# AIM-SE/AC-TSR

Hardware: AMD Instinct MI355X
Metric: user-sequences/sec fwd+bwd, AC-SASRec L=50 d=64, 1/2/4/8 MI355X (higher is better)
Workload: dtype f32; 1 GPU; ACSASRec full training step (spatial + adversarial calibrators, BASELINE configs[2]), synthetic 100000-item catalogue, B=512/GPU L=50 d=64 h=2 2 layers inner=256, CE loss, two-pass backward + Adam; global_batch=512, seq_len=50, hidden=64, heads=2, parallelism=dp1, launch=hipGraph replay per step, backward=two walks (reference protocol, trainer.py:672-686)

## Files before the change

### ac_tsr_amd/_lib.py

```python
from __future__ import annotations

import ctypes as C
import os
import subprocess

_HERE = os.path.dirname(os.path.abspath(__file__))
CSRC = os.path.join(_HERE, "csrc")
LIB_PATH = os.environ.get("ACATTN_LIB") or os.path.join(CSRC, "libacattn.so")
HEADER_PATH = os.path.join(os.path.dirname(_HERE), "include", "acattn.h")

ABI_VERSION = 29
MAX_MASKS = 8
NSTAT = 8
MASK_STRUCTURED, MASK_DENSE_LL, MASK_DENSE_L = 0, 1, 2
COMBINE = {"fixed": 0, "gate": 1, "annealing": 2}
RICH = {"none": 0, "fixed": 1, "trainable": 2}
RNG_EXPLICIT, RNG_COUNTER = 0, 1
FWD_AUTO, FWD_STREAM, FWD_STAGED, FWD_GENERAL = 0, 1, 2, 3
BWD_AUTO, BWD_STREAM, BWD_ROW = 0, 1, 2

_f = C.c_void_p


class Problem(C.Structure):
    _fields_ = [
        ("B", C.c_int32), ("L", C.c_int32), ("H", C.c_int32), ("n_heads", C.c_int32),
        ("q", _f), ("k", _f), ("v", _f), ("qa", _f), ("ka", _f), ("gate_logits", _f),
        ("mask_mode", C.c_int32), ("causal", C.c_int32), ("key_valid", _f), ("mask", _f),
        ("w_order", _f), ("b_order", _f), ("w_dist", _f), ("b_dist", _f), ("scalar", _f),
        ("adversarial", C.c_int32), ("combine_option", C.c_int32), ("anneal_rate", C.c_float),
        ("two_level", C.c_int32), ("rich_combine", C.c_int32), ("rich_ratio", _f),
        ("rng_mode", C.c_int32), ("p_drop", C.c_float), ("noise", _f), ("keep_after", _f), ("keep_before", _f),
        ("keep_mask", _f), ("seed", C.c_uint64), ("seed_device", _f), ("affine", _f), ("gate_is_prob", C.c_int32),
    ]


class FwdOut(C.Structure):
    _fields_ = [
        ("ctx_attacked", _f), ("ctx_calibrated", _f), ("attack_mask", _f), ("row_stats", _f),
        ("after_spatial", _f), ("before_spatial", _f), ("perturbed_attention", _f), ("calibrated_attention", _f),
        ("penalty_part", _f),
    ]


# ... 63 lines not shown


class TailBwdIO(C.Structure):
    _fields_ = [("d_out", _f), ("d_ctx", _f), ("d_x", _f), ("d_h1", _f), ("d_h2", _f), ("d_h3", _f), ("dgb_part", _f),
                ("workspace", _f)]


class EmbedProblem(C.Structure):
    _fields_ = [("rows", C.c_int32), ("L", C.c_int32), ("H", C.c_int32), ("n_table_rows", C.c_int64), ("idx", _f),
                ("table", _f), ("pos", _f), ("gamma", _f), ("beta", _f), ("eps", C.c_float), ("p_drop", C.c_float),
                ("keep", _f), ("seed", C.c_uint64), ("seed_device", _f), ("nonzero_out", _f), ("hot_id_plus1", C.c_int64)]


EMBED_BWD_CHUNKS = 8
PENALTY_WS_FLOATS = 1024
WGRAD_MAX_GROUP = 8
WGRAD_MAX_REDUCE = 32
SUMROWS_MAX_DEFER = 8

SYMBOLS = {
    "acattn_abi_version": (C.c_int, []),
    "acattn_calibrated_attention_bwd_gate_summed": (C.c_int, [C.POINTER(Problem), C.POINTER(BwdIO)]),
    "acattn_calibrated_attention_bwd_pair_supported": (C.c_int, [C.POINTER(Problem), C.POINTER(BwdIO)]),
    "acattn_last_error": (C.c_char_p, []),
    "acattn_fwd_algorithmic_bytes": (C.c_int64, [C.POINTER(Problem)]),
    "acattn_calibrated_attention_fwd": (C.c_int, [C.POINTER(Problem), C.POINTER(FwdOut), C.c_void_p]),
    "acattn_calibrated_attention_bwd": (C.c_int, [C.POINTER(Problem), C.POINTER(BwdIO), C.c_void_p]),
    "acattn_spatial_affines": (C.c_int, [C.POINTER(Problem), _f, C.c_void_p]),
    "acattn_full_sort_ce_workspace_bytes": (C.c_int64, [C.POINTER(CeProblem)]),
    "acattn_full_sort_ce_fwd": (C.c_int, [C.POINTER(CeProblem), _f, _f, _f, C.c_void_p]),
    "acattn_full_sort_ce_fwd_dir": (C.c_int, [C.POINTER(CeProblem), _f, _f, _f, _f, C.c_void_p]),
    "acattn_full_sort_ce_bwd": (C.c_int, [C.POINTER(CeProblem), _f, _f, _f, _f, _f, C.c_void_p]),
    "acattn_full_sort_ce_products": (C.c_int, [C.c_int]),
    "acattn_dropout_add_layernorm_fwd": (C.c_int, [C.POINTER(LnProblem), _f, _f, C.c_void_p]),
    "acattn_dropout_add_layernorm_bwd": (C.c_int, [C.POINTER(LnProblem), _f, _f, _f, _f, _f, C.c_void_p]),
    "acattn_embed_layernorm_fwd": (C.c_int, [C.POINTER(EmbedProblem), _f, _f, C.c_void_p]),
    "acattn_embed_layernorm_bwd": (C.c_int, [C.POINTER(EmbedProblem), _f, _f, C.c_int64, _f, _f, _f, C.c_void_p]),
    "acattn_projections_supported": (C.c_int, [C.c_int32, C.c_int32]),
    "acattn_projections_bwd_workspace_bytes": (C.c_int64, [C.POINTER(ProjProblem)]),
    "acattn_projections_fwd": (C.c_int, [C.POINTER(ProjProblem), C.POINTER(ProjOut), C.c_void_p]),
    "acattn_projections_bwd": (C.c_int, [C.POINTER(ProjProblem), C.POINTER(ProjBwdIO), C.c_void_p]),
    "acattn_layer_tail_supported": (C.c_int, [C.c_int32, C.c_int32]),
    "acattn_layer_tail_fwd": (C.c_int, [C.POINTER(TailProblem), C.POINTER(TailSaved), C.c_void_p]),
    "acattn_layer_tail_bwd": (C.c_int, [C.POINTER(TailProblem), C.POINTER(TailSaved), C.POINTER(TailBwdIO), C.c_void_p]),
    "acattn_layer_tail_bwd_partial_rows": (C.c_int32, [C.c_int32]),
    "acattn_layer_tail_bwd_partial_rows_for": (C.c_int32, [C.c_int32, C.c_int32]),
    "acattn_layer_tail_bwd_workspace_bytes": (C.c_int64, [C.c_int32, C.c_int32]),
    "acattn_select_layer_tail_blocks": (C.c_int, [C.c_int]),
    "acattn_adam_step": (C.c_int, [C.POINTER(AdamGroup), C.c_double, C.c_double, C.c_double, C.c_double, C.c_double, _f,
                                   C.c_void_p]),
    "acattn_dense_ce_fwd": (C.c_int, [_f, C.c_int64, C.c_int64, _f, _f, _f, C.c_void_p]),
    "acattn_dense_ce_bwd": (C.c_int, [_f, _f, _f, _f, C.c_int64, C.c_int64, _f, C.c_void_p]),
    "acattn_step_inputs": (C.c_int, [C.POINTER(C.c_void_p), C.POINTER(C.c_void_p), C.POINTER(C.c_int64), C.c_int32, C.c_void_p,
                                     C.c_void_p, C.c_void_p, C.c_int32, C.c_void_p]),
    "acattn_sum_rows": (C.c_int, [_f, _f, C.c_int32, C.c_int32, C.c_int32, C.c_void_p]),
    "acattn_sum_rows_pair": (C.c_int, [_f, _f, C.c_int32, C.c_int32, C.c_int32, _f, _f, C.c_int32, C.c_int32, C.c_int32, C.c_void_p]),
    "acattn_mask_penalty_fwd": (C.c_int, [_f, C.c_int64, _f, _f, C.c_void_p]),
    "acattn_mask_penalty_partial": (C.c_int, [_f, C.c_int64, _f, C.c_void_p]),
    "acattn_mask_penalty_partial_multi": (C.c_int, [C.c_void_p, C.c_int32, C.c_int64, _f, C.c_void_p]),
    "acattn_mask_penalty_bwd_scaled_multi": (C.c_int, [C.c_void_p, _f, _f, C.c_float, C.c_int64, C.c_void_p, C.c_int32,
                                                       C.c_void_p]),
    "acattn_attacked_loss_finish": (C.c_int, [_f, C.c_int32, _f, C.c_int32, C.c_int64, C.c_float, _f, _f, C.c_int32,
                                              C.c_void_p]),
    "acattn_mask_penalty_rows": (C.c_int, [_f, C.c_int32, C.c_int32, C.c_int32, _f, C.c_void_p]),
    "acattn_attacked_loss_finish_rows": (C.c_int, [_f, C.c_int32, C.c_void_p, C.c_int32, C.c_int32, C.c_float, _f, _f, C.c_int32,
                                                  C.c_void_p]),
# ... 65 lines not shown
```

### ac_tsr_amd/csrc/acattn_api.hip

```cpp
#include <stdint.h>
#include <stdio.h>
#include <string.h>

#include <algorithm>

#include "acattn_common.h"

namespace {
thread_local char g_err[256] = "";

int fail(const char* msg) {
  snprintf(g_err, sizeof(g_err), "%s", msg);
  return -1;
}

int check_problem(const acattn_problem* p) {
  if (!p) return fail("problem is NULL");
  if (p->B < 1 || p->L < 1 || p->H < 1 || p->n_heads < 1) return fail("B, L, H, n_heads must be positive");
  if (p->H % p->n_heads != 0)
    return fail("The hidden size is not a multiple of the number of attention heads");
  const int dh = p->H / p->n_heads;
  if (dh != 16 && dh != 32 && dh != 64 && dh != 128) return fail("unsupported head size: dh must be 16, 32, 64 or 128");
  if (p->L > 208) return fail("unsupported sequence length: L must be <= 208");
  if (!p->q || !p->k || !p->v) return fail("q, k, v must be non-NULL");
// ... 126 lines not shown
int64_t acattn_full_sort_ce_workspace_bytes(const acattn_ce_problem* p) {
  if (!p || (p->H != 64 && p->H != 128 && p->H != 256)) return -1;
  return acattn_ce_ws_bytes(*p);
}

int acattn_full_sort_ce_fwd(const acattn_ce_problem* p, void* workspace, float* lse, float* row_loss, void* stream) {
  if (int rc = check_ce(p)) return rc;
  if (!workspace || !lse || !row_loss) return fail("workspace, lse, row_loss must be non-NULL");
  const int rc = acattn_launch_ce_fwd(*p, workspace, lse, row_loss, (hipStream_t)stream);
  if (rc > 0) snprintf(g_err, sizeof(g_err), "HIP launch failed: %s", hipGetErrorString((hipError_t)rc));
  return rc;
}

int acattn_full_sort_ce_fwd_dir(const acattn_ce_problem* p, void* workspace, float* lse, float* row_loss, float* dir,
                                void* stream) {
  if (int rc = check_ce(p)) return rc;
  if (!workspace || !lse || !row_loss || !dir) return fail("workspace, lse, row_loss, dir must be non-NULL");
  const int rc = acattn_launch_ce_fwd_dir(*p, workspace, lse, row_loss, dir, (hipStream_t)stream);
  if (rc > 0) snprintf(g_err, sizeof(g_err), "HIP launch failed: %s", hipGetErrorString((hipError_t)rc));
  return rc;
}

int acattn_full_sort_ce_bwd(const acattn_ce_problem* p, const float* lse, const float* coef, void* workspace,
                            float* d_out, float* d_table, void* stream) {
  if (int rc = check_ce(p)) return rc;
  if (!workspace || !lse || !coef || !d_out) return fail("workspace, lse, coef, d_out must be non-NULL");
  const int rc = acattn_launch_ce_bwd(*p, lse, coef, workspace, d_out, d_table, (hipStream_t)stream);
  if (rc > 0) snprintf(g_err, sizeof(g_err), "HIP launch failed: %s", hipGetErrorString((hipError_t)rc));
  return rc;
}

int acattn_full_sort_ce_products(int mode) { return acattn_ce_products_choice(mode); }

static int check_ln(const acattn_ln_problem* p) {
  if (!p) return fail("ln problem is NULL");
  if (p->rows < 1) return fail("rows must be positive");
  if (p->H != 64 && p->H != 128 && p->H != 256) return fail("unsupported hidden size for the fused LayerNorm: H must be 64, 128 or 256");
  if (p->residual_rows < 1 || p->rows % p->residual_rows != 0) return fail("residual_rows must divide rows");
  if (!p->z || !p->residual || !p->gamma || !p->beta) return fail("z, residual, gamma, beta must be non-NULL");
  if (p->p_drop < 0.f || p->p_drop >= 1.f) return fail("p_drop must lie in [0, 1)");
  return 0;
}

int acattn_dropout_add_layernorm_fwd(const acattn_ln_problem* p, float* y, float* stats, void* stream) {
  if (int rc = check_ln(p)) return rc;
  if (!y || !stats) return fail("y and stats must be non-NULL");
  const int rc = acattn_launch_ln_fwd(*p, y, stats, (hipStream_t)stream);
  if (rc > 0) snprintf(g_err, sizeof(g_err), "HIP launch failed: %s", hipGetErrorString((hipError_t)rc));
  return rc;
}

int acattn_dropout_add_layernorm_bwd(const acattn_ln_problem* p, const float* dy, const float* stats, float* dz,
                                     float* dres, float* dgb_part, void* stream) {
  if (int rc = check_ln(p)) return rc;
  if (!dy || !stats) return fail("dy and stats must be non-NULL");
  const int rc = acattn_launch_ln_bwd(*p, dy, stats, dz, dres, dgb_part, (hipStream_t)stream);
  if (rc > 0) snprintf(g_err, sizeof(g_err), "HIP launch failed: %s", hipGetErrorString((hipError_t)rc));
  return rc;
}

static int check_proj(const acattn_proj_problem* p) {
  if (!p) return fail("problem must be non-NULL");
  if (p->rows < 1) return fail("rows must be positive");
  if (!acattn_proj_supported(p->H, p->G)) return fail("projections: hidden_size must be 64, 128 or 256 and the gate at most 256 wide");
  if (!p->x || !p->wq || !p->bq || !p->wk || !p->bk || !p->wv || !p->bv || !p->waq || !p->baq || !p->wak || !p->bak)
    return fail("projections: input and parameters must be non-NULL");
// ... 363 lines not shown
```

### ac_tsr_amd/csrc/acattn_ce_bf16.hip

```cpp
#include <stdlib.h>

#include "acattn_common.h"

namespace {

constexpr float kLog2e = 1.44269504088896340736f;
constexpr float kLn2 = 0.69314718055994530942f;
constexpr int CH = 64;
constexpr int NW = 4;
constexpr int ES = CH + 4;
constexpr int HSLOTS = 24;
constexpr int HB_BYTES = HSLOTS * 64 * 16;
#ifndef CE6_EC_AGPR
#define CE6_EC_AGPR 1
#endif
#ifndef CE6_PIPE
#define CE6_PIPE 0
#endif

typedef __bf16 b8 __attribute__((ext_vector_type(8)));
typedef __bf16 b4 __attribute__((ext_vector_type(4)));
typedef short s4v __attribute__((ext_vector_type(4)));
typedef short s8v __attribute__((ext_vector_type(8)));

#define CE6_TERMS(X) X(0, 2) X(1, 1) X(2, 0) X(0, 1) X(1, 0) X(0, 0)

__device__ __forceinline__ f4 mfma_bf(const b8 a, const b8 b, const f4 c) {
  return __builtin_amdgcn_mfma_f32_16x16x32_bf16(a, b, c, 0, 0, 0);
}

__device__ __forceinline__ void dma16(const void* gsrc, void* lds_dst) {
  const uint32_t lds_off = (uint32_t)(uintptr_t)(__attribute__((address_space(3))) char*)lds_dst;
  asm volatile("s_mov_b32 m0, %1\n\ts_nop 0\n\tglobal_load_lds_dwordx4 %0, off" ::"v"(gsrc), "s"(lds_off) : "memory", "m0");
}

__device__ __forceinline__ void split8(const float (&x)[8], b8& p0, b8& p1, b8& p2) {
#pragma unroll
  for (int j = 0; j < 8; ++j) {
    const __bf16 a = (__bf16)x[j];
    const float r1 = x[j] - (float)a;
    const __bf16 b = (__bf16)r1;
    const float r2 = r1 - (float)b;
    p0[j] = a;
    p1[j] = b;
    p2[j] = (__bf16)r2;
  }
}

__global__ void __launch_bounds__(256) ce_split_rows_kernel(const float* __restrict__ out, const int B, b8* __restrict__ Hb,
                                                            float* __restrict__ zero, const int64_t n_zero) {
  const int sb = blockIdx.x;
  for (int64_t i = (int64_t)blockIdx.x * 256 + threadIdx.x; i < n_zero; i += (int64_t)gridDim.x * 256) zero[i] = 0.f;
  for (int e = threadIdx.x; e < 8 * 64; e += 256) {
    const int grp = e >> 6, lane = e & 63, c = lane & 15, g = lane >> 4;
    float x[8];
    if (grp < 4) {
      const int row = 32 * sb + 16 * (grp >> 1) + c;
      f4 v0 = {0.f, 0.f, 0.f, 0.f}, v1 = v0;
      if (row < B) {
        v0 = *(const f4*)(out + (size_t)row * CH + 32 * (grp & 1) + 8 * g);
        v1 = *(const f4*)(out + (size_t)row * CH + 32 * (grp & 1) + 8 * g + 4);
      }
#pragma unroll
      for (int j = 0; j < 4; ++j) {
        x[j] = v0[j];
        x[4 + j] = v1[j];
      }
    } else {
#pragma unroll
      for (int j = 0; j < 8; ++j) {
        const int row = 32 * sb + 8 * g + j;
        x[j] = row < B ? out[(size_t)row * CH + 16 * (grp - 4) + c] : 0.f;
      }
    }
    b8 p[3];
    split8(x, p[0], p[1], p[2]);
#pragma unroll
    for (int q = 0; q < 3; ++q) {
      const int slot = grp < 4 ? grp * 3 + q : 12 + 4 * q + (grp - 4);
// ... 828 lines not shown
```

### ac_tsr_amd/csrc/acattn_common.h

```cpp
#pragma once
#include <hip/hip_runtime.h>
#include <stdint.h>

#include <type_traits>

#include "acattn.h"

typedef float f4 __attribute__((ext_vector_type(4)));
typedef float f4u __attribute__((ext_vector_type(4), aligned(4)));

#define ACATTN_NEG_INF (-__builtin_inff())
#define ACATTN_MASK_FILL (-10000.0f)
#define ACATTN_LOG_EPS (1e-24f)

__device__ __forceinline__ float quad_sum(float x) {
  auto r = __builtin_amdgcn_permlane16_swap(__float_as_uint(x), __float_as_uint(x), false, false);
  x = __uint_as_float(r[0]) + __uint_as_float(r[1]);
  auto s = __builtin_amdgcn_permlane32_swap(__float_as_uint(x), __float_as_uint(x), false, false);
  return __uint_as_float(s[0]) + __uint_as_float(s[1]);
}

__device__ __forceinline__ float quad_max(float x) {
  auto r = __builtin_amdgcn_permlane16_swap(__float_as_uint(x), __float_as_uint(x), false, false);
  x = fmaxf(__uint_as_float(r[0]), __uint_as_float(r[1]));
// ... 268 lines not shown
int acattn_launch_linear_wgrad(const float* const* x, const float* const* dy, const int* K, const int* N,
                               float* const* dw, float* const* db, int n_items, int64_t M, void* ws, hipStream_t stream,
                               int* P_out = nullptr, long long* w_off_out = nullptr, long long* b_off_out = nullptr);
int acattn_launch_linear_wgrad_reduce_many(const float* const* part_w, const float* const* part_b, const int* K, const int* N,
                                           const int* P, float* const* dw, float* const* db, int n_items,
                                           const float* const* sr_x, float* const* sr_out, const int* sr_R, const int* sr_C,
                                           int n_sr, hipStream_t stream);
int acattn_launch_embed_fwd(const acattn_embed_problem& p, float* y, float* stats, hipStream_t stream);
int acattn_launch_embed_bwd(const acattn_embed_problem& p, const float* dy, const float* stats, int64_t padding_idx,
                            float* d_table, float* d_pos_part, float* dgb_part, hipStream_t stream);
int acattn_launch_penalty_fwd(const float* m, int64_t n, float* ws, float* norm, hipStream_t stream);
int acattn_launch_penalty_partial(const float* m, int64_t n, float* part, hipStream_t stream);
void acattn_penalty_written_set(bool v);
bool acattn_penalty_written();
int acattn_launch_penalty_rows(const float* m, int B, int nh, int L, float* pen, hipStream_t stream);
int acattn_launch_attacked_loss_finish_rows(const float* row_loss, int B, const float* const* pen, int n_masks, int count,
                                            float weight, float* out, float* scale_buf, int n_scale, hipStream_t stream);
int acattn_launch_penalty_drows(const float* norms, const float* d_loss, float scale, int count, float* const* d_pen,
                                int n_masks, hipStream_t stream, const float* dir = nullptr, float* d_out = nullptr, int n_dir = 0);
int acattn_launch_attacked_loss_finish(const float* row_loss, int B, const float* part, int n_masks, int64_t mask_numel,
                                       float weight, float* out, float* scale_buf, int n_scale, hipStream_t stream);
int acattn_launch_penalty_bwd_scaled(const float* m, const float* norm, const float* d_loss, float scale, int64_t n,
                                     float* d_m, hipStream_t stream);
int acattn_launch_penalty_bwd(const float* m, const float* norm, const float* d_norm, int64_t n, float* d_m,
                              hipStream_t stream);
int acattn_launch_zero(float* p, size_t n, hipStream_t stream);
int64_t acattn_ce6_rows_bytes(const acattn_ce_problem& p);
int acattn_launch_ce6_sweep(const acattn_ce_problem& p, const float* lse, const float* coef, float* slab, float* d_table,
                            float2* part, void* rows_ws, int n_wg, int n_left, bool dir, hipStream_t stream);
int acattn_launch_ce6_onehot_reduce(const acattn_ce_problem& p, const float* coef, const float* slab, int n_slabs, float* d_out,
                                    float* d_table, hipStream_t stream);
int acattn_launch_ce6_fwd_sweep(const acattn_ce_problem& p, float2* part, void* rows_ws, int n_wg, int n_left, hipStream_t stream);
int acattn_ce_products_choice(int mode);
int acattn_launch_dense_ce_fwd(const float* logits, int64_t rows, int64_t N, const int64_t* target, float* lse, float* row_loss,
                               hipStream_t stream);
int acattn_launch_dense_ce_bwd(const float* logits, const float* lse, const int64_t* target, const float* coef, int64_t rows,
                               int64_t N, float* d_logits, hipStream_t stream);
int acattn_launch_step_inputs(const void* const* src, void* const* dst, const int64_t* bytes, int n, int64_t* counter,
                              const int64_t* item_length, int64_t* last_row, int n_rows, hipStream_t stream);
int acattn_launch_penalty_partial_multi(const float* const* m, int n_masks, int64_t n, float* part, hipStream_t stream);
int acattn_launch_penalty_bwd_scaled_multi(const float* const* m, const float* norms, const float* d_loss, float scale,
                                           int64_t n, float* const* d_m, int n_masks, hipStream_t stream);
int acattn_launch_adam_step(const acattn_adam_group& g, double lr, double beta1, double beta2, double eps,
                            double weight_decay, int* done, hipStream_t stream);
```

### ac_tsr_amd/csrc/acattn_proj.hip

```cpp
#include <stdlib.h>

#include <algorithm>
#include <type_traits>

#include "acattn_common.h"
#include "acattn_wstage.h"

namespace {

template <int NB>
struct Rows {
  int row[NB];
  bool ok[NB];
};

template <int NB>
__device__ __forceinline__ Rows<NB> wave_rows(int R) {
  Rows<NB> w;
  const int c = threadIdx.x & 15;
#pragma unroll
  for (int nb = 0; nb < NB; ++nb) {
    const int r = (blockIdx.x * NB + nb) * 16 + c;
    w.ok[nb] = r < R;
    w.row[nb] = r < R ? r : R - 1;
  }
  return w;
}

template <int DT>
__device__ __forceinline__ void load_weight(const float* w, int H, int n_out, int c, int g, f4 (&frag)[DT][DT]) {
#pragma unroll
  for (int nt = 0; nt < DT; ++nt) {
    const int o = min(16 * nt + c, n_out - 1);
#pragma unroll
    for (int t = 0; t < DT; ++t) frag[nt][t] = *(const f4*)(w + (size_t)o * H + 16 * t + 4 * g);
  }
}

// ... 784 lines not shown
#pragma unroll
          for (int nt = 0; nt < KT; ++nt)
#pragma unroll
            for (int nb = 0; nb < NB; ++nb) {
              if (half == 0) tot[nb][nt] = mfma16(frag[nt][r], d[nb][r], tot[nb][nt]);
              else tot[nb][DT - KT + nt] = mfma16(frag[nt][r], d[nb][r], tot[nb][DT - KT + nt]);
            }
        PIN_ORDER();
        st.commit();
      }
    }
  }
  if (h_qt) masked_store_rows(IO.dmq_total, tot);
  if (h_dmk) load_rows<DT, NB>(IO.dmk, W, g, tot); else zero(tot);
  if (h_dka) {
    load_rows<DT, NB>(IO.dka, W, g, in);
    staged_keep<DT, NB, false>(st, wakT, nullptr, in, tot, after_k_total);
  }
  if (h_kt) masked_store_rows(IO.dmk_total, tot);
  if (h_dx) {
    f4 (&dx)[NB][DT] = in;
    if (IO.dx_init) load_rows<DT, NB>(IO.dx_init, W, g, dx); else zero(dx);
    staged_keep<DT, NB, false>(st, wkT, nullptr, tot, dx, [&] { first(wqT); });
    load_rows<DT, NB>(IO.dmq_total, W, g, tot);
    staged_keep<DT, NB, false>(st, wqT, nullptr, tot, dx, [&] { if (h_dmv) first(wvT); else st.has_bias = false; });
    if (h_dmv) {
      load_rows<DT, NB>(IO.dmv, W, g, tot);
      staged_keep<DT, NB, false>(st, wvT, nullptr, tot, dx, [&] { st.has_bias = false; });
    }
    masked_store_rows(IO.dx, dx);
  }
}

int rows_per_wave(int rows) {
  static const int forced = getenv("ACATTN_PROJ_ROWS_PER_WAVE") ? atoi(getenv("ACATTN_PROJ_ROWS_PER_WAVE")) : 0;
  if (forced == 16 || forced == 32) return forced;
  return rows >= 16384 ? 32 : 16;
}

}

bool acattn_proj_supported(int H, int G) { return (H == 64 || H == 128 || H == 256) && G >= 0 && G <= 256; }

int64_t acattn_proj_bwd_ws_bytes(const acattn_proj_problem& p) {
  if (p.H == 64) return 0;
  return ((int64_t)5 * p.H * p.H + (int64_t)p.H * ((p.G + 15) & ~15)) * (int64_t)sizeof(float);
}

namespace {
template <int H>
int launch_wide_fwd(const acattn_proj_problem& p, const acattn_proj_out& o, hipStream_t stream) {
#ifdef ACATTN_PROJ_NB1
  constexpr int NB = 1;
#else
  constexpr int NB = H == 128 ? 2 : 1;
#endif
  static const bool per_wave = getenv("ACATTN_PROJ_PER_WAVE") != nullptr;
  if (!per_wave) {
    const int blocks = (p.rows + 16 * NB * NWV - 1) / (16 * NB * NWV);
    hipLaunchKernelGGL((proj_staged_fwd_kernel<H, NB>), dim3(blocks), dim3(64 * NWV), 0, stream, p, o);
    return (int)hipGetLastError();
  }
  const int blocks = (p.rows + 16 * NB - 1) / (16 * NB);
  hipLaunchKernelGGL((proj_wide_fwd_kernel<H, NB>), dim3(blocks), dim3(64), 0, stream, p, o);
  return (int)hipGetLastError();
}
// ... 13 lines not shown
  const float* src[6] = {p.wq, p.wk, p.wv, p.waq, p.wak, p.wg};
  for (int k = 0; k < 6; ++k) {
    J.src[k] = src[k];
    J.n_out[k] = k < 5 ? p.H : p.G;
  }
  const int max_out = std::max(p.H, (p.G + 15) & ~15);
  hipLaunchKernelGGL(transpose_weights_kernel, dim3(max_out / 16, p.H / 16, p.wg ? 6 : 5), dim3(256), 0, stream, J, p.H, wt);
  const bool outs = io.dx && io.dmq_total && io.dmk_total, attack = io.dqa && io.dka;
  const bool all_in = attack && io.dmq && io.dmk && io.dmv && (io.dgate || !p.wg);
  const bool attack_only = attack && !io.dmq && !io.dmk && !io.dmv && !io.dgate;
  const int mode = !outs ? 0 : all_in ? 1 : attack_only ? 2 : 0;
  static const bool per_wave = getenv("ACATTN_PROJ_PER_WAVE") != nullptr;
  if (!per_wave) {
    const int wgs = (p.rows + 16 * NB * NWV - 1) / (16 * NB * NWV);
    if (mode == 1)
      hipLaunchKernelGGL((proj_staged_bwd_kernel<H, NB, 1>), dim3(wgs), dim3(64 * NWV), 0, stream, p, io, (const float*)wt);
    else if (mode == 2)
      hipLaunchKernelGGL((proj_staged_bwd_kernel<H, NB, 2>), dim3(wgs), dim3(64 * NWV), 0, stream, p, io, (const float*)wt);
    else
      hipLaunchKernelGGL((proj_staged_bwd_kernel<H, NB, 0>), dim3(wgs), dim3(64 * NWV), 0, stream, p, io, (const float*)wt);
    return (int)hipGetLastError();
  }
  const int blocks = (p.rows + 16 * NB - 1) / (16 * NB);
  if (mode == 1)
    hipLaunchKernelGGL((proj_wide_bwd_kernel<H, NB, 1>), dim3(blocks), dim3(64), 0, stream, p, io, (const float*)wt);
  else if (mode == 2)
    hipLaunchKernelGGL((proj_wide_bwd_kernel<H, NB, 2>), dim3(blocks), dim3(64), 0, stream, p, io, (const float*)wt);
  else
    hipLaunchKernelGGL((proj_wide_bwd_kernel<H, NB, 0>), dim3(blocks), dim3(64), 0, stream, p, io, (const float*)wt);
  return (int)hipGetLastError();
}
}

int acattn_launch_proj_fwd(const acattn_proj_problem& p, const acattn_proj_out& o, hipStream_t stream) {
  if (p.H == 128) return launch_wide_fwd<128>(p, o, stream);
  if (p.H == 256) return launch_wide_fwd<256>(p, o, stream);
  const int rpw = rows_per_wave(p.rows), blocks = (p.rows + rpw - 1) / rpw;
  if (rpw == 32)
    hipLaunchKernelGGL((proj_fwd_kernel<64, 2>), dim3(blocks), dim3(64), 0, stream, p, o);
  else
    hipLaunchKernelGGL((proj_fwd_kernel<64, 1>), dim3(blocks), dim3(64), 0, stream, p, o);
  return (int)hipGetLastError();
}

int acattn_launch_proj_bwd(const acattn_proj_problem& p, const acattn_proj_bwd_io& io, hipStream_t stream) {
  if (p.H == 128) return launch_wide_bwd<128>(p, io, stream);
  if (p.H == 256) return launch_wide_bwd<256>(p, io, stream);
  const int rpw = rows_per_wave(p.rows), blocks = (p.rows + rpw - 1) / rpw;
  const bool outs = io.dx && io.dmq_total && io.dmk_total, attack = io.dqa && io.dka;
  const bool all_in = attack && io.dmq && io.dmk && io.dmv && (io.dgate || !p.wg);
  const bool attack_only = attack && !io.dmq && !io.dmk && !io.dmv && !io.dgate;
  const int mode = !outs ? 0 : all_in ? 1 : attack_only ? 2 : 0;
#define LAUNCH(NB, MODE) hipLaunchKernelGGL((proj_bwd_kernel<64, NB, MODE>), dim3(blocks), dim3(64), 0, stream, p, io)
  if (rpw == 32) {
    if (mode == 1) LAUNCH(2, 1); else if (mode == 2) LAUNCH(2, 2); else LAUNCH(2, 0);
  } else {
    if (mode == 1) LAUNCH(1, 1); else if (mode == 2) LAUNCH(1, 2); else LAUNCH(1, 0);
  }
#undef LAUNCH
  return (int)hipGetLastError();
}
```

### include/acattn.h

```cpp
#ifndef ACATTN_H_
#define ACATTN_H_

#include <stdint.h>

#ifdef __cplusplus
extern "C" {
#endif

#define ACATTN_ABI_VERSION 29

enum {
  ACATTN_MASK_STRUCTURED = 0,
  ACATTN_MASK_DENSE_LL = 1,
  ACATTN_MASK_DENSE_L = 2
};

enum { ACATTN_COMBINE_FIXED = 0, ACATTN_COMBINE_GATE = 1, ACATTN_COMBINE_ANNEALING = 2 };

enum { ACATTN_RICH_NONE = 0, ACATTN_RICH_FIXED = 1, ACATTN_RICH_TRAINABLE = 2 };

enum {
  ACATTN_RNG_EXPLICIT = 0,
  ACATTN_RNG_COUNTER = 1
};

#define ACATTN_NSTAT 8

typedef struct acattn_problem {
  int32_t B, L, H, n_heads;
  const float* q;
  const float* k;
  const float* v;
  const float* qa;
  const float* ka;
  const float* gate_logits;
  int32_t mask_mode;
  int32_t causal;
  const uint8_t* key_valid;
  const float* mask;
  const float* w_order;
  const float* b_order;
  const float* w_dist;
// ... 236 lines not shown
typedef struct acattn_proj_problem {
  int32_t rows, H, G;
  const float* x;
  const float *wq, *bq;
  const float *wk, *bk;
  const float *wv, *bv;
  const float *waq, *baq;
  const float *wak, *bak;
  const float *wg, *bg;
  const float *w_order, *b_order, *w_dist, *b_dist;
  int32_t n_heads, L;
} acattn_proj_problem;

typedef struct acattn_proj_out {
  float *mq, *mk, *mv, *qa, *ka;
  float* gate;
  float* affine;
  int32_t gate_prob;
} acattn_proj_out;

typedef struct acattn_proj_bwd_io {
  const float *dmq, *dmk, *dmv, *dqa, *dka;
  const float* dgate;
  float *dmq_total, *dmk_total, *dx;
  const float* dx_init;
  void* workspace;
} acattn_proj_bwd_io;

int acattn_projections_supported(int32_t H, int32_t G);
int64_t acattn_projections_bwd_workspace_bytes(const acattn_proj_problem* p);
int acattn_projections_fwd(const acattn_proj_problem* p, const acattn_proj_out* out, void* stream);
int acattn_projections_bwd(const acattn_proj_problem* p, const acattn_proj_bwd_io* io, void* stream);

#define ACATTN_ADAM_MAX_TENSORS 64
typedef struct acattn_adam_group {
  int32_t n_tensors;
  float* param[ACATTN_ADAM_MAX_TENSORS];
  const float* grad[ACATTN_ADAM_MAX_TENSORS];
  float* exp_avg[ACATTN_ADAM_MAX_TENSORS];
  float* exp_avg_sq[ACATTN_ADAM_MAX_TENSORS];
  float* step[ACATTN_ADAM_MAX_TENSORS];
  int64_t numel[ACATTN_ADAM_MAX_TENSORS];
} acattn_adam_group;
int acattn_adam_step(const acattn_adam_group* g, double lr, double beta1, double beta2, double eps, double weight_decay,
                     int32_t* done, void* stream);

int acattn_calibrated_attention_bwd_gate_summed(const acattn_problem* p, const acattn_bwd_io* io);
int acattn_calibrated_attention_bwd_pair_supported(const acattn_problem* p, const acattn_bwd_io* io);

int acattn_abi_version(void);

const char* acattn_last_error(void);

int64_t acattn_fwd_algorithmic_bytes(const acattn_problem* p);

int acattn_calibrated_attention_fwd(const acattn_problem* p, const acattn_fwd_out* out, void* stream);

int acattn_spatial_affines(const acattn_problem* p, float* affine, void* stream);

int acattn_calibrated_attention_bwd(const acattn_problem* p, const acattn_bwd_io* io, void* stream);

int64_t acattn_calibrated_attention_bwd_workspace_bytes(const acattn_problem* p);

int acattn_rng_materialize(int32_t B, int32_t n_heads, int32_t L, uint64_t seed, float p_drop, float* noise,
                           uint8_t* keep_after, uint8_t* keep_mask, uint8_t* keep_before, void* stream);

// ... 20 lines not shown
```

Before: 472,100 user-sequences/sec.

## Use split-bf16 MFMA products for H=64 attention projection kernels

Result: faster. 479,700 user-sequences/sec, median of 6 (+1.6%).

```diff
diff --git a/ac_tsr_amd/_lib.py b/ac_tsr_amd/_lib.py
--- a/ac_tsr_amd/_lib.py
+++ b/ac_tsr_amd/_lib.py
@@ -9,7 +9,7 @@
 LIB_PATH = os.environ.get("ACATTN_LIB") or os.path.join(CSRC, "libacattn.so")
 HEADER_PATH = os.path.join(os.path.dirname(_HERE), "include", "acattn.h")
 
-ABI_VERSION = 29
+ABI_VERSION = 30
 MAX_MASKS = 8
 NSTAT = 8
 MASK_STRUCTURED, MASK_DENSE_LL, MASK_DENSE_L = 0, 1, 2
@@ -139,6 +139,7 @@
     "acattn_full_sort_ce_fwd_dir": (C.c_int, [C.POINTER(CeProblem), _f, _f, _f, _f, C.c_void_p]),
     "acattn_full_sort_ce_bwd": (C.c_int, [C.POINTER(CeProblem), _f, _f, _f, _f, _f, C.c_void_p]),
     "acattn_full_sort_ce_products": (C.c_int, [C.c_int]),
+    "acattn_linear_products": (C.c_int, [C.c_int]),
     "acattn_dropout_add_layernorm_fwd": (C.c_int, [C.POINTER(LnProblem), _f, _f, C.c_void_p]),
     "acattn_dropout_add_layernorm_bwd": (C.c_int, [C.POINTER(LnProblem), _f, _f, _f, _f, _f, C.c_void_p]),
     "acattn_embed_layernorm_fwd": (C.c_int, [C.POINTER(EmbedProblem), _f, _f, C.c_void_p]),
diff --git a/ac_tsr_amd/csrc/acattn_api.hip b/ac_tsr_amd/csrc/acattn_api.hip
--- a/ac_tsr_amd/csrc/acattn_api.hip
+++ b/ac_tsr_amd/csrc/acattn_api.hip
@@ -182,6 +182,8 @@
 
 int acattn_full_sort_ce_products(int mode) { return acattn_ce_products_choice(mode); }
 
+int acattn_linear_products(int mode) { return acattn_linear_products_choice(mode); }
+
 static int check_ln(const acattn_ln_problem* p) {
   if (!p) return fail("ln problem is NULL");
   if (p->rows < 1) return fail("rows must be positive");
diff --git a/ac_tsr_amd/csrc/acattn_ce_bf16.hip b/ac_tsr_amd/csrc/acattn_ce_bf16.hip
--- a/ac_tsr_amd/csrc/acattn_ce_bf16.hip
+++ b/ac_tsr_amd/csrc/acattn_ce_bf16.hip
@@ -1,6 +1,7 @@
 #include <stdlib.h>
 
 #include "acattn_common.h"
+#include "acattn_split.h"
 
 namespace {
 
@@ -18,33 +19,15 @@
 #define CE6_PIPE 0
 #endif
 
-typedef __bf16 b8 __attribute__((ext_vector_type(8)));
 typedef __bf16 b4 __attribute__((ext_vector_type(4)));
 typedef short s4v __attribute__((ext_vector_type(4)));
 typedef short s8v __attribute__((ext_vector_type(8)));
 
-#define CE6_TERMS(X) X(0, 2) X(1, 1) X(2, 0) X(0, 1) X(1, 0) X(0, 0)
-
-__device__ __forceinline__ f4 mfma_bf(const b8 a, const b8 b, const f4 c) {
-  return __builtin_amdgcn_mfma_f32_16x16x32_bf16(a, b, c, 0, 0, 0);
-}
+#define CE6_TERMS(X) ACATTN_SPLIT_TERMS(X)
 
 __device__ __forceinline__ void dma16(const void* gsrc, void* lds_dst) {
   const uint32_t lds_off = (uint32_t)(uintptr_t)(__attribute__((address_space(3))) char*)lds_dst;
   asm volatile("s_mov_b32 m0, %1\n\ts_nop 0\n\tglobal_load_lds_dwordx4 %0, off" ::"v"(gsrc), "s"(lds_off) : "memory", "m0");
-}
-
-__device__ __forceinline__ void split8(const float (&x)[8], b8& p0, b8& p1, b8& p2) {
-#pragma unroll
-  for (int j = 0; j < 8; ++j) {
-    const __bf16 a = (__bf16)x[j];
-    const float r1 = x[j] - (float)a;
-    const __bf16 b = (__bf16)r1;
-    const float r2 = r1 - (float)b;
-    p0[j] = a;
-    p1[j] = b;
-    p2[j] = (__bf16)r2;
-  }
 }
 
 __global__ void __launch_bounds__(256) ce_split_rows_kernel(const float* __restrict__ out, const int B, b8* __restrict__ Hb,
diff --git a/ac_tsr_amd/csrc/acattn_common.h b/ac_tsr_amd/csrc/acattn_common.h
--- a/ac_tsr_amd/csrc/acattn_common.h
+++ b/ac_tsr_amd/csrc/acattn_common.h
@@ -324,6 +324,7 @@
                                     float* d_table, hipStream_t stream);
 int acattn_launch_ce6_fwd_sweep(const acattn_ce_problem& p, float2* part, void* rows_ws, int n_wg, int n_left, hipStream_t stream);
 int acattn_ce_products_choice(int mode);
+int acattn_linear_products_choice(int mode);
 int acattn_launch_dense_ce_fwd(const float* logits, int64_t rows, int64_t N, const int64_t* target, float* lse, float* row_loss,
                                hipStream_t stream);
 int acattn_launch_dense_ce_bwd(const float* logits, const float* lse, const int64_t* target, const float* coef, int64_t rows,
diff --git a/ac_tsr_amd/csrc/acattn_proj.hip b/ac_tsr_amd/csrc/acattn_proj.hip
--- a/ac_tsr_amd/csrc/acattn_proj.hip
+++ b/ac_tsr_amd/csrc/acattn_proj.hip
@@ -1,9 +1,11 @@
 #include <stdlib.h>
+#include <string.h>
 
 #include <algorithm>
 #include <type_traits>
 
 #include "acattn_common.h"
+#include "acattn_split.h"
 #include "acattn_wstage.h"
 
 namespace {
@@ -854,6 +856,246 @@
   }
 }
 
+constexpr int SPW = 4;
+constexpr int SPLIT_MAT = 4 * 2 * 3 * 64;
+constexpr int SPLIT_LDS = 6 * SPLIT_MAT * (int)sizeof(b8);
+
+__device__ __forceinline__ int kperm(int s, int g, int j) { return 32 * s + 16 * (j >> 2) + 4 * g + (j & 3); }
+
+template <bool T>
+__device__ __forceinline__ void split_raw(const float* w, int n_out, int nt, int c, int g, float (&v)[2][8]) {
+#pragma unroll
+  for (int s = 0; s < 2; ++s) {
+    if constexpr (!T) {
+      const float* row = w + (size_t)min(16 * nt + c, n_out - 1) * 64 + 32 * s + 4 * g;
+      const f4 lo = *(const f4*)row, hi = *(const f4*)(row + 16);
+#pragma unroll
+      for (int r = 0; r < 4; ++r) {
+        v[s][r] = lo[r];
+        v[s][4 + r] = hi[r];
+      }
+    } else {
+#pragma unroll
+      for (int j = 0; j < 8; ++j) {
+        const int k = kperm(s, g, j);
+        const float t = w[(size_t)min(k, n_out - 1) * 64 + 16 * nt + c];
+        v[s][j] = k < n_out ? t : 0.f;
+      }
+    }
+  }
+}
+
+__device__ __forceinline__ void split_store(const float (&v)[2][8], b8* mat, int nt, int lane) {
+#pragma unroll
+  for (int s = 0; s < 2; ++s) {
+    b8 p[3];
+    split8(v[s], p[0], p[1], p[2]);
+#pragma unroll
+    for (int q = 0; q < 3; ++q) mat[((nt * 2 + s) * 3 + q) * 64 + lane] = p[q];
+  }
+}
+
+template <int NB>
+__device__ __forceinline__ void split_rows(const f4 (&v)[NB][4], b8 (&b)[NB][2][3]) {
+#pragma unroll
+  for (int nb = 0; nb < NB; ++nb)
+#pragma unroll
+    for (int s = 0; s < 2; ++s) {
+      float x[8];
+#pragma unroll
+      for (int r = 0; r < 4; ++r) {
+        x[r] = v[nb][2 * s][r];
+        x[4 + r] = v[nb][2 * s + 1][r];
+      }
+      split8(x, b[nb][s][0], b[nb][s][1], b[nb][s][2]);
+    }
+}
+
+template <int NB, int NT = 4>
+__device__ __forceinline__ void split_product(const b8* mat, int lane, const b8 (&b)[NB][2][3], f4 (&acc)[NB][4]) {
+#pragma unroll
+  for (int nt = 0; nt < NT; ++nt) {
+    b8 a[2][3];
+#pragma unroll
+    for (int s = 0; s < 2; ++s)
+#pragma unroll
+      for (int q = 0; q < 3; ++q) a[s][q] = mat[((nt * 2 + s) * 3 + q) * 64 + lane];
+#pragma unroll
+    for (int s = 0; s < 2; ++s)
+#pragma unroll
+      for (int nb = 0; nb < NB; ++nb) acc[nb][nt] = mfma_split(a[s], b[nb][s], acc[nb][nt]);
+  }
+}
+
+template <int NB>
+__device__ __forceinline__ Rows<NB> split_rows_of(int R, int wave) {
+  Rows<NB> w;
+  const int c = threadIdx.x & 15;
+#pragma unroll
+  for (int nb = 0; nb < NB; ++nb) {
+    const int r = ((blockIdx.x * SPW + wave) * NB + nb) * 16 + c;
+    w.ok[nb] = r < R;
+    w.row[nb] = r < R ? r : R - 1;
+  }
+  return w;
+}
+
+template <int NB>
+__global__ void __launch_bounds__(64 * SPW) proj_split_fwd_kernel(const acattn_proj_problem P, const acattn_proj_out O) {
+  extern __shared__ b8 wsp[];
+  const int lane = threadIdx.x & 63, wave = threadIdx.x >> 6, c = lane & 15, g = lane >> 4;
+  const Rows<NB> W = split_rows_of<NB>(P.rows, wave);
+  const bool gate = P.wg != nullptr;
+  {
+    const float* src[6] = {P.wq, P.waq, gate ? P.wg : P.wq, P.wk, P.wak, P.wv};
+    float v[6][2][8];
+#pragma unroll
+    for (int m = 0; m < 6; ++m) split_raw<false>(src[m], m == 2 && gate ? P.G : 64, wave, c, g, v[m]);
+#pragma unroll
+    for (int m = 0; m < 6; ++m)
+      if (m != 2 || gate) split_store(v[m], wsp + m * SPLIT_MAT, wave, lane);
+  }
+  f4 xb[NB][4], m[NB][4], acc[NB][4];
+  b8 xs[NB][2][3], ms[NB][2][3];
+  f4 bias[4];
+  load_rows<4, NB>(P.x, W, g, xb);
+  load_bias<4>(P.bq, g, bias);
+  __syncthreads();
+  split_rows<NB>(xb, xs);
+  set_rows<4, NB>(bias, m);
+  split_product<NB>(wsp, lane, xs, m);
+  store_rows<4, NB>(O.mq, W, g, m);
+  if (O.affine) write_affine<4, NB>(m, W, P, O.affine, 0, P.b_order[0], P.b_dist[0], 0, c, g);
+  split_rows<NB>(m, ms);
+  load_bias<4>(P.baq, g, bias);
+  set_rows<4, NB>(bias, acc);
+  split_product<NB>(wsp + SPLIT_MAT, lane, ms, acc);
+  store_rows<4, NB>(O.qa, W, g, acc);
+  if (gate) {
+    const int GT = (P.G + 15) >> 4;
+#pragma unroll
+    for (int nt = 0; nt < 4; ++nt) {
+      f4 b;
+#pragma unroll
+      for (int r = 0; r < 4; ++r) b[r] = P.bg[min(16 * nt + 4 * g + r, P.G - 1)];
+#pragma unroll
+      for (int nb = 0; nb < NB; ++nb) acc[nb][nt] = b;
+    }
+    split_product<NB>(wsp + 2 * SPLIT_MAT, lane, ms, acc);
+#pragma unroll
+    for (int nt = 0; nt < 4; ++nt) {
+      if (nt >= GT) break;
+#pragma unroll
+      for (int nb = 0; nb < NB; ++nb) {
+        f4 v = acc[nb][nt];
+        if (O.gate_prob) v = gate_value(v, 0);
+        const int j0 = 16 * nt + 4 * g;
+        float* dst = O.gate + (size_t)W.row[nb] * P.G + j0;
+        if (W.ok[nb] && j0 + 3 < P.G) {
+          *(f4u*)dst = v;
+        } else if (W.ok[nb]) {
+#pragma unroll
+          for (int r = 0; r < 4; ++r)
+            if (j0 + r < P.G) dst[r] = v[r];
+        }
+      }
+    }
+  }
+  load_bias<4>(P.bk, g, bias);
+  set_rows<4, NB>(bias, m);
+  split_product<NB>(wsp + 3 * SPLIT_MAT, lane, xs, m);
+  store_rows<4, NB>(O.mk, W, g, m);
+  if (O.affine) write_affine<4, NB>(m, W, P, O.affine, 64 / P.n_heads, 0.f, 0.f, 2, c, g);
+  split_rows<NB>(m, ms);
+  load_bias<4>(P.bak, g, bias);
+  set_rows<4, NB>(bias, acc);
+  split_product<NB>(wsp + 4 * SPLIT_MAT, lane, ms, acc);
+  store_rows<4, NB>(O.ka, W, g, acc);
+  load_bias<4>(P.bv, g, bias);
+  set_rows<4, NB>(bias, acc);
+  split_product<NB>(wsp + 5 * SPLIT_MAT, lane, xs, acc);
+  store_rows<4, NB>(O.mv, W, g, acc);
+}
+
+template <int NB, int MODE>
+__global__ void __launch_bounds__(64 * SPW) proj_split_bwd_kernel(const acattn_proj_problem P, const acattn_proj_bwd_io IO) {
+  extern __shared__ b8 wsp[];
+  const bool h_dmq = MODE == 1 || (MODE == 0 && IO.dmq), h_dmk = MODE == 1 || (MODE == 0 && IO.dmk);
+  const bool h_dmv = MODE == 1 || (MODE == 0 && IO.dmv);
+  const bool h_dqa = MODE != 0 || IO.dqa, h_dka = MODE != 0 || IO.dka, h_dx = MODE != 0 || IO.dx;
+  const bool h_qt = MODE != 0 || IO.dmq_total, h_kt = MODE != 0 || IO.dmk_total;
+  const bool gate = MODE != 2 && IO.dgate && P.wg;
+  const int lane = threadIdx.x & 63, wave = threadIdx.x >> 6, c = lane & 15, g = lane >> 4;
+  const Rows<NB> W = split_rows_of<NB>(P.rows, wave);
+  {
+    const float* src[6] = {P.waq, gate ? P.wg : P.waq, P.wq, P.wak, P.wk, P.wv};
+    const bool need[6] = {h_dqa, gate, h_dx, h_dka, h_dx, h_dx && h_dmv};
+    float v[6][2][8];
+#pragma unroll
+    for (int m = 0; m < 6; ++m)
+      if (need[m]) split_raw<true>(src[m], m == 1 ? P.G : 64, wave, c, g, v[m]);
+#pragma unroll
+    for (int m = 0; m < 6; ++m)
+      if (need[m]) split_store(v[m], wsp + m * SPLIT_MAT, wave, lane);
+  }
+  auto zero = [&](f4 (&v)[NB][4]) {
+#pragma unroll
+    for (int nb = 0; nb < NB; ++nb)
+#pragma unroll
+      for (int t = 0; t < 4; ++t) v[nb][t] = f4{0.f, 0.f, 0.f, 0.f};
+  };
+  f4 in[NB][4], dq[NB][4], dk[NB][4], dx[NB][4];
+  b8 bs[NB][2][3];
+  if (IO.dx_init && h_dx) load_rows<4, NB>(IO.dx_init, W, g, dx); else zero(dx);
+  if (h_dmq) load_rows<4, NB>(IO.dmq, W, g, dq); else zero(dq);
+  if (h_dqa) load_rows<4, NB>(IO.dqa, W, g, in);
+  __syncthreads();
+
+  if (h_dqa) {
+    split_rows<NB>(in, bs);
+    split_product<NB>(wsp, lane, bs, dq);
+  }
+  if (gate) {
+#pragma unroll
+    for (int nb = 0; nb < NB; ++nb)
+#pragma unroll
+      for (int s = 0; s < 2; ++s) {
+        float x[8];
+#pragma unroll
+        for (int j = 0; j < 8; ++j) {
+          const int k = kperm(s, g, j);
+          const float t = IO.dgate[(size_t)W.row[nb] * P.G + min(k, P.G - 1)];
+          x[j] = k < P.G ? t : 0.f;
+        }
+        split8(x, bs[nb][s][0], bs[nb][s][1], bs[nb][s][2]);
+      }
+    split_product<NB>(wsp + SPLIT_MAT, lane, bs, dq);
+  }
+  if (h_qt) store_rows<4, NB>(IO.dmq_total, W, g, dq);
+  if (h_dx) {
+    split_rows<NB>(dq, bs);
+    split_product<NB>(wsp + 2 * SPLIT_MAT, lane, bs, dx);
+  }
+
+  if (h_dmk) load_rows<4, NB>(IO.dmk, W, g, dk); else zero(dk);
+  if (h_dka) {
+    load_rows<4, NB>(IO.dka, W, g, in);
+    split_rows<NB>(in, bs);
+    split_product<NB>(wsp + 3 * SPLIT_MAT, lane, bs, dk);
+  }
+  if (h_kt) store_rows<4, NB>(IO.dmk_total, W, g, dk);
+  if (h_dx) {
+    split_rows<NB>(dk, bs);
+    split_product<NB>(wsp + 4 * SPLIT_MAT, lane, bs, dx);
+    if (h_dmv) {
+      load_rows<4, NB>(IO.dmv, W, g, in);
+      split_rows<NB>(in, bs);
+      split_product<NB>(wsp + 5 * SPLIT_MAT, lane, bs, dx);
+    }
+    store_rows<4, NB>(IO.dx, W, g, dx);
+  }
+}
+
 int rows_per_wave(int rows) {
   static const int forced = getenv("ACATTN_PROJ_ROWS_PER_WAVE") ? atoi(getenv("ACATTN_PROJ_ROWS_PER_WAVE")) : 0;
   if (forced == 16 || forced == 32) return forced;
@@ -933,10 +1175,52 @@
 }
 }
 
+namespace {
+int g_linear_products = -1;
+int linear_products() {
+  if (g_linear_products < 0) {
+    const char* e = getenv("ACATTN_LINEAR_PRODUCTS");
+    g_linear_products = e && !strcmp(e, "fp32") ? 0 : 1;
+  }
+  return g_linear_products;
+}
+bool use_split(const acattn_proj_problem& p) { return p.H == 64 && (!p.wg || p.G <= 64) && linear_products() == 1; }
+
+template <class K>
+bool allow_split_lds(K kern) {
+  return hipFuncSetAttribute((const void*)kern, hipFuncAttributeMaxDynamicSharedMemorySize, SPLIT_LDS) == hipSuccess;
+}
+
+template <int NB>
+int launch_split_fwd(const acattn_proj_problem& p, const acattn_proj_out& o, hipStream_t stream) {
+  static const bool lds_ok = allow_split_lds(proj_split_fwd_kernel<NB>);
+  if (!lds_ok) return (int)hipErrorInvalidValue;
+  const int wgs = (p.rows + 16 * NB * SPW - 1) / (16 * NB * SPW);
+  hipLaunchKernelGGL((proj_split_fwd_kernel<NB>), dim3(wgs), dim3(64 * SPW), SPLIT_LDS, stream, p, o);
+  return (int)hipGetLastError();
+}
+
+template <int NB, int MODE>
+int launch_split_bwd(const acattn_proj_problem& p, const acattn_proj_bwd_io& io, hipStream_t stream) {
+  static const bool lds_ok = allow_split_lds(proj_split_bwd_kernel<NB, MODE>);
+  if (!lds_ok) return (int)hipErrorInvalidValue;
+  const int wgs = (p.rows + 16 * NB * SPW - 1) / (16 * NB * SPW);
+  hipLaunchKernelGGL((proj_split_bwd_kernel<NB, MODE>), dim3(wgs), dim3(64 * SPW), SPLIT_LDS, stream, p, io);
+  return (int)hipGetLastError();
+}
+}
+
+int acattn_linear_products_choice(int mode) {
+  const int old = linear_products();
+  if (mode >= 0 && mode <= 1) g_linear_products = mode;
+  return old;
+}
+
 int acattn_launch_proj_fwd(const acattn_proj_problem& p, const acattn_proj_out& o, hipStream_t stream) {
   if (p.H == 128) return launch_wide_fwd<128>(p, o, stream);
   if (p.H == 256) return launch_wide_fwd<256>(p, o, stream);
   const int rpw = rows_per_wave(p.rows), blocks = (p.rows + rpw - 1) / rpw;
+  if (use_split(p)) return rpw == 32 ? launch_split_fwd<2>(p, o, stream) : launch_split_fwd<1>(p, o, stream);
   if (rpw == 32)
     hipLaunchKernelGGL((proj_fwd_kernel<64, 2>), dim3(blocks), dim3(64), 0, stream, p, o);
   else
@@ -952,6 +1236,16 @@
   const bool all_in = attack && io.dmq && io.dmk && io.dmv && (io.dgate || !p.wg);
   const bool attack_only = attack && !io.dmq && !io.dmk && !io.dmv && !io.dgate;
   const int mode = !outs ? 0 : all_in ? 1 : attack_only ? 2 : 0;
+  if (use_split(p)) {
+    if (rpw == 32) {
+      if (mode == 1) return launch_split_bwd<2, 1>(p, io, stream);
+      if (mode == 2) return launch_split_bwd<2, 2>(p, io, stream);
+      return launch_split_bwd<2, 0>(p, io, stream);
+    }
+    if (mode == 1) return launch_split_bwd<1, 1>(p, io, stream);
+    if (mode == 2) return launch_split_bwd<1, 2>(p, io, stream);
+    return launch_split_bwd<1, 0>(p, io, stream);
+  }
 #define LAUNCH(NB, MODE) hipLaunchKernelGGL((proj_bwd_kernel<64, NB, MODE>), dim3(blocks), dim3(64), 0, stream, p, io)
   if (rpw == 32) {
     if (mode == 1) LAUNCH(2, 1); else if (mode == 2) LAUNCH(2, 2); else LAUNCH(2, 0);
diff --git a/ac_tsr_amd/csrc/acattn_split.h b/ac_tsr_amd/csrc/acattn_split.h
--- /dev/null
+++ b/ac_tsr_amd/csrc/acattn_split.h
@@ -0,0 +1,35 @@
+#pragma once
+
+#include "acattn_common.h"
+
+namespace {
+
+typedef __bf16 b8 __attribute__((ext_vector_type(8)));
+
+#define ACATTN_SPLIT_TERMS(X) X(0, 2) X(1, 1) X(2, 0) X(0, 1) X(1, 0) X(0, 0)
+
+__device__ __forceinline__ f4 mfma_bf(const b8 a, const b8 b, const f4 c) {
+  return __builtin_amdgcn_mfma_f32_16x16x32_bf16(a, b, c, 0, 0, 0);
+}
+
+__device__ __forceinline__ void split8(const float (&x)[8], b8& p0, b8& p1, b8& p2) {
+#pragma unroll
+  for (int j = 0; j < 8; ++j) {
+    const __bf16 a = (__bf16)x[j];
+    const float r1 = x[j] - (float)a;
+    const __bf16 b = (__bf16)r1;
+    const float r2 = r1 - (float)b;
+    p0[j] = a;
+    p1[j] = b;
+    p2[j] = (__bf16)r2;
+  }
+}
+
+__device__ __forceinline__ f4 mfma_split(const b8 (&a)[3], const b8 (&b)[3], f4 acc) {
+#define ACATTN_SPLIT_TERM(p, q) acc = mfma_bf(a[p], b[q], acc);
+  ACATTN_SPLIT_TERMS(ACATTN_SPLIT_TERM)
+#undef ACATTN_SPLIT_TERM
+  return acc;
+}
+
+}
diff --git a/include/acattn.h b/include/acattn.h
--- a/include/acattn.h
+++ b/include/acattn.h
@@ -7,7 +7,7 @@
 extern "C" {
 #endif
 
-#define ACATTN_ABI_VERSION 29
+#define ACATTN_ABI_VERSION 30
 
 enum {
   ACATTN_MASK_STRUCTURED = 0,
@@ -310,6 +310,10 @@
 int acattn_projections_fwd(const acattn_proj_problem* p, const acattn_proj_out* out, void* stream);
 int acattn_projections_bwd(const acattn_proj_problem* p, const acattn_proj_bwd_io* io, void* stream);
 
+#define ACATTN_LINEAR_PRODUCTS_FP32 0
+#define ACATTN_LINEAR_PRODUCTS_DEFAULT 1
+int acattn_linear_products(int mode);
+
 #define ACATTN_ADAM_MAX_TENSORS 64
 typedef struct acattn_adam_group {
   int32_t n_tensors;
```
